# tonyzyl/ladcast

Measured on AMD Instinct MI355X. Metric: ensemble-member-steps/sec, higher is better.
Workload: dtype f32

## Files before the change

### ladcast_amd/csrc/gemm_bf16x3_v3.hip

```cpp
#include <math.h>
#include <stdio.h>
#include <stdlib.h>

#include "common.h"

namespace {

#include "gemm_v3_common.inc"
#include "gemm_v3_kstep_f32.inc"

struct SKArgs {
  DevProblem pr[MAXP];
  int np;
  int G;
  long long U;
  long long tiles;
  float* ws;
  unsigned* counters;
  unsigned upg, urem;
};

__device__ __forceinline__ long long range_start(long long g, const SKArgs& a) {
  const unsigned gu = static_cast<unsigned>(g);
  return static_cast<long long>(gu * a.upg + (gu < a.urem ? gu : a.urem));
}

__device__ __forceinline__ int find_problem_by_unit(const SKArgs& a, long long u) {
  int pi = 0;
#pragma unroll
  for (int k = 1; k < MAXP; ++k)
    if (k < a.np && u >= a.pr[k].unit0) pi = k;
  return pi;
}

#ifdef LDC_GEMM_STAMPS
#define LDC_STAMP(i)                                                                                        \
  if (threadIdx.x == 0)                                                                                     \
    reinterpret_cast<unsigned long long*>(a.counters)[65536 + blockIdx.x * 16 + (i)] = __builtin_amdgcn_s_memrealtime();
#define LDC_STAMP_CLK(i)                                                                                    \
  if (threadIdx.x == 0)                                                                                     \
    reinterpret_cast<unsigned long long*>(a.counters)[65536 + blockIdx.x * 16 + (i)] = __builtin_amdgcn_s_memtime();
#else
#define LDC_STAMP(i)
#define LDC_STAMP_CLK(i)
#endif

template <int BM, int TERMS, bool CONV = false>
__global__ __launch_bounds__(512) void gemm_bf16x3_v3_kernel(SKArgs a) {
  constexpr int CPK = TERMS == 1 ? 2 * BK : BK;
  constexpr int RT = BM / 128;
  constexpr int NACC = RT * 8;
  constexpr int STAGE_B = (BM + BN) * ROW_B;
  constexpr int SLOT_FLOATS = BM * BN;
  constexpr int NAI = BM / 64;
  constexpr int ND = NAI + 2;
  constexpr int NDH = ND / 2;
  extern __shared__ __attribute__((aligned(16))) unsigned char smem[];
  const int wave = __builtin_amdgcn_readfirstlane(static_cast<int>(threadIdx.x) >> 6);
  LDC_STAMP(0)
  int seg_ = 0;
  (void)seg_;
  int g;
  {
    const int bid = blockIdx.x, G = a.G;
    const int q = G >> 3, r = G & 7, xcd = bid & 7;
    g = (xcd < r ? xcd * (q + 1) : r * (q + 1) + (xcd - r) * q) + (bid >> 3);
  }
  auto uniform64 = [](long long v) {
    const unsigned lo = __builtin_amdgcn_readfirstlane(static_cast<unsigned>(v));
    const unsigned hi = __builtin_amdgcn_readfirstlane(static_cast<unsigned>(static_cast<unsigned long long>(v) >> 32));
    return static_cast<long long>((static_cast<unsigned long long>(hi) << 32) | lo);
  };
  const long long u_begin = uniform64(range_start(g, a));
  const long long u_end = uniform64(range_start(g + 1, a));
  const unsigned smem_lds = lds_addr(smem);

  struct Seg {
    int pi, tile, k0, k1, b, bm, bn;
  };
  auto decode = [&](long long u_) {
    Seg sg;
    sg.pi = find_problem_by_unit(a, u_);
    const DevProblem& Q = a.pr[sg.pi];
    const unsigned local = static_cast<unsigned>(u_ - Q.unit0), kt_u = static_cast<unsigned>(Q.kt);
    sg.tile = __builtin_amdgcn_readfirstlane(static_cast<int>(local / kt_u));
    sg.k0 = static_cast<int>(local - static_cast<unsigned>(sg.tile) * kt_u);
    const long long left = u_end - u_;
    sg.k1 = (Q.kt - sg.k0 <= left) ? Q.kt : sg.k0 + static_cast<int>(left);
    const unsigned per_b = static_cast<unsigned>(Q.tm * Q.tn), tile_u = static_cast<unsigned>(sg.tile);
    const unsigned b_ = tile_u / per_b;
    const unsigned t_in = tile_u - b_ * per_b;
    const unsigned strip = static_cast<unsigned>(Q.rm * Q.tn);
    const unsigned sr = t_in / strip;
    const unsigned r_in = t_in - sr * strip;
    const int rest = Q.tm - static_cast<int>(sr) * Q.rm;
    const unsigned h_sr = static_cast<unsigned>(rest < Q.rm ? rest : Q.rm);
    const unsigned bn_ = r_in / h_sr;
    sg.b = __builtin_amdgcn_readfirstlane(static_cast<int>(b_));
    sg.bn = __builtin_amdgcn_readfirstlane(static_cast<int>(bn_));
    sg.bm = __builtin_amdgcn_readfirstlane(static_cast<int>(sr) * Q.rm + static_cast<int>(r_in - bn_ * h_sr));
    return sg;
  };
  auto prefetch_next = [&](const Seg& sg) __attribute__((always_inline)) {
    const DevProblem& Q = a.pr[sg.pi];
    const int ln = fresh_lane();
    const int lr_ = ln >> 3, lp_ = ln & 7;
    const float* __restrict__ An = Q.A + static_cast<long long>(sg.b) * Q.d.a_bs;
    const long long wrb = static_cast<long long>(Q.d.K) * (TERMS == 1 ? 2 : 4);
    unsigned char* dump = smem + NSTAGE * STAGE_B + wave * 1024;
#pragma unroll
    for (int j = 0; j < 2; ++j) {
      const bool live = sg.k0 + j < sg.k1;
      const long long koff = static_cast<long long>(live ? sg.k0 + j : sg.k1 - 1) * (BK * 4);
      unsigned char* sA = smem + j * STAGE_B;
      unsigned char* sW = sA + BM * ROW_B;
#pragma unroll
      for (int i = 0; i < NAI; ++i) {
        const int r = 8 * (wave + 8 * i) + lr_;
        int gm = sg.bm * BM + r;
        gm = gm < Q.d.M ? gm : Q.d.M - 1;
        dma16(reinterpret_cast<const unsigned char*>(An + static_cast<long long>(gm) * Q.d.lda) + ((lp_ ^ swz(r)) << 4) + koff,
              live ? sA + (wave + 8 * i) * 1024 : dump);
      }
#pragma unroll
      for (int i = 0; i < 2; ++i) {
        const int r = 8 * (wave + 8 * i) + lr_;
        int gn = sg.bn * BN + r;
        gn = gn < Q.d.N ? gn : Q.d.N - 1;
        dma16(Q.W + static_cast<long long>(gn) * wrb + ((lp_ ^ swz(r)) << 4) + koff, live ? sW + (wave + 8 * (i)) * 1024 : dump);
      }
    }
  };
  long long u = u_begin;
  Seg cur{};
  if (u < u_end) cur = decode(u);
  bool prefetched = false;
  while (u < u_end) {
    const int pi = cur.pi;
    const DevProblem& P = a.pr[pi];
    const int tile = cur.tile, k0 = cur.k0, k1 = cur.k1, b = cur.b, bm = cur.bm, bn = cur.bn;
    const int lane = fresh_lane();
    const int fr = lane & 15;
    const int kg = lane >> 4;
    const int lr = lane >> 3, lp = lane & 7;
    const unsigned f_r = swz(fr);
    const unsigned off_hi = fr * ROW_B + (((2 * kg) ^ f_r) << 4);
    const unsigned off_lo = fr * ROW_B + (((2 * kg + 1) ^ f_r) << 4);
    const unsigned a_hi = smem_lds + (16 * RT * wave) * ROW_B + off_hi;
    const unsigned a_lo = smem_lds + (16 * RT * wave) * ROW_B + off_lo;
    const unsigned w_hi = smem_lds + BM * ROW_B + off_hi;
    const unsigned w_lo = smem_lds + BM * ROW_B + off_lo;
    const int M = P.d.M, N = P.d.N, K = P.d.K;
    const bool wave_rows = bm * BM + 16 * RT * wave < M;
    const float* __restrict__ A = P.A + static_cast<long long>(b) * P.d.a_bs;
    const int lda = P.d.lda;
    const long long w_row_bytes = static_cast<long long>(K) * (TERMS == 1 ? 2 : 4);

#ifdef LDC_GEMM_STAMPS_PROLOGUE
    if (seg_ == 0) { LDC_STAMP(9) }
#endif
    const unsigned char* a_src[NAI];
    const unsigned char* w_src[2];
    int pix_b[NAI], pix_hw[NAI];
    const int cslot = lp ^ swz(8 * (wave & 1) + lr);
    auto conv_tap_base = [&](int i, int tap) {
      const int ky = tap / P.ks, kx = tap - ky * P.ks;
      const int src = pix_b[i] + ldc_sphere_src_pixel(pix_hw[i] >> 16, pix_hw[i] & 0xffff, ky, kx, P.cH, P.cW, P.ks);
      return reinterpret_cast<const unsigned char*>(A + static_cast<long long>(src) * lda) + (cslot << 4);
    };
#pragma unroll
    for (int i = 0; i < NAI; ++i) {
      const int r = 8 * (wave + 8 * i) + lr;
      int gm = bm * BM + r;
      gm = gm < M ? gm : M - 1;
      if constexpr (CONV) {
        const int hw = P.cH * P.cW;
        const int bimg = gm / hw;
        const int rem = gm - bimg * hw;
        const int h = rem / P.cW;
        pix_b[i] = bimg * hw;
        pix_hw[i] = (h << 16) | (rem - h * P.cW);
        a_src[i] = conv_tap_base(i, k0 >> P.kshift);
      } else {
        a_src[i] = reinterpret_cast<const unsigned char*>(A + static_cast<long long>(gm) * lda) + ((lp ^ swz(r)) << 4);
      }
    }
#pragma unroll
    for (int i = 0; i < 2; ++i) {
      const int r = 8 * (wave + 8 * i) + lr;
      int gn = bn * BN + r;
      gn = gn < N ? gn : N - 1;
      w_src[i] = P.W + static_cast<long long>(gn) * w_row_bytes + ((lp ^ swz(r)) << 4);
    }
    auto issue_one = [&](int kt_, int stage, int i) {
      const bool live = kt_ < k1;
      unsigned char* sA = smem + stage * STAGE_B;
      unsigned char* sW = sA + BM * ROW_B;
      unsigned char* dump = smem + NSTAGE * STAGE_B + wave * 1024;
      const int kt = live ? kt_ : k1 - 1;
      const long long koff = static_cast<long long>(kt) * (BK * 4);
#ifdef LDC_GEMM_DIAG_NODMA
      if (kt >= 0) return;
#endif
      if (i < NAI) {
        if constexpr (CONV) {
          const int chunk = kt & ((1 << P.kshift) - 1);
          if (chunk == 0) a_src[i] = conv_tap_base(i, kt >> P.kshift);
          const unsigned char* src = a_src[i] + chunk * (BK * 4);
          if (chunk * CPK + CPK > P.cin) {
            if (chunk * CPK + (TERMS == 0 ? 4 * cslot : 8 * (TERMS == 3 ? (cslot >> 1) : cslot)) >= P.cin) src = P.zero16;
          }
          dma16(src, live ? sA + (wave + 8 * i) * 1024 : dump);
        } else {
          dma16(a_src[i] + koff, live ? sA + (wave + 8 * i) * 1024 : dump);
        }
      } else {
        dma16(w_src[i - NAI] + koff, live ? sW + (wave + 8 * (i - NAI)) * 1024 : dump);
      }
    };

// ... 77 lines not shown
    const unsigned sb1 = st1 * STAGE_B;                                                                      \
    const unsigned wch = w_hi + sb, wcl = w_lo + sb, wnh = w_hi + sb1, wnl = w_lo + sb1;                     \
    const unsigned anh = a_hi + sb1, anl = a_lo + sb1;                                                       \
    constexpr bool dma2 = true;              \
    constexpr bool dma3 = true;  \
        \
    if constexpr (RT == 2) {                                                                                 \
      asm volatile("s_waitcnt lgkmcnt(6)" : "+v"(AH[0]), "+v"(AL[0]), "+v"(AH[1]), "+v"(AL[1]), "+v"(wh0), "+v"(wl0)); \
    } else {                                                                                                 \
      asm volatile("s_waitcnt lgkmcnt(6)" : "+v"(AH[0]), "+v"(AL[0]), "+v"(wh0), "+v"(wl0));                 \
    }                                                                                                        \
    LDC_SB;                                                                                                  \
    LDC_CT(0, wh0, wl0, AH, AL)                                                                              \
    LDC_RD_W(wh0, wl0, wch, wcl, 4)                                                                                \
    if (dma2) issue_one(kt + 2, st2, NDH + 0);                                                               \
    LDC_WAIT(6, wh1, wl1)                                                                                    \
    LDC_CT(1, wh1, wl1, AH, AL)                                                                              \
    LDC_RD_W(wh1, wl1, wch, wcl, 5)                                                                                \
    if (dma2) issue_one(kt + 2, st2, NDH + 1);                                                               \
    LDC_WAIT(6, wh2, wl2)                                                                                    \
    LDC_CT(2, wh2, wl2, AH, AL)                                                                              \
    LDC_RD_W(wh2, wl2, wch, wcl, 6)                                                                                \
    if constexpr (NDH == 3) {                                                                                \
      if (dma2) issue_one(kt + 2, st2, NDH + 2);                                                             \
    }                                                                                                        \
    LDC_WAIT(6, wh3, wl3)                                                                                    \
    LDC_CT(3, wh3, wl3, AH, AL)                                                                              \
    LDC_RD_W(wh3, wl3, wch, wcl, 7)                                                                          \
    LDC_WAIT(6, wh0, wl0)                                                                                    \
    LDC_CT(4, wh0, wl0, AH, AL)                                                                              \
                                                                         \
    asm volatile("s_waitcnt lgkmcnt(0)" : "+v"(wh1), "+v"(wl1), "+v"(wh2), "+v"(wl2), "+v"(wh3), "+v"(wl3)); \
    if constexpr (ND == 6) {                                                                                 \
      asm volatile("s_waitcnt vmcnt(6)" ::: "memory");                                                       \
    } else {                                                                                                 \
      asm volatile("s_waitcnt vmcnt(4)" ::: "memory");                                                       \
    }                                                                                                        \
    LDC_KSTEP_BARRIER                                                                                        \
    LDC_SB;                                                                                                  \
                          \
    LDC_RD_A(AHN, ALN, anh, anl)                                                                             \
    LDC_RD_W(wh0, wl0, wnh, wnl, 0)                                                                          \
    if (dma3) issue_one(kt + 3, st, 0);                                                                      \
    LDC_SB;                                                                                                  \
    LDC_CT(5, wh1, wl1, AH, AL)                                                                              \
    LDC_RD_W(wh1, wl1, wnh, wnl, 1)                                                                               \
    if (dma3) issue_one(kt + 3, st, 1);                                                                      \
    LDC_SB;                                                                                                  \
    LDC_CT(6, wh2, wl2, AH, AL)                                                                              \
    LDC_RD_W(wh2, wl2, wnh, wnl, 2)                                                                               \
    if constexpr (NDH == 3) {                                                                                \
      if (dma3) issue_one(kt + 3, st, 2);                                                                    \
    }                                                                                                        \
    LDC_SB;                                                                                                  \
    LDC_CT(7, wh3, wl3, AH, AL)                                                                              \
    LDC_RD_W(wh3, wl3, wnh, wnl, 3)                                                                               \
    LDC_SB;                                                                                                  \
    st = st1;                                                                                                \
    sb = sb1;                                                                                                \
  }

#define LDC_MM_ON(ACC, WF, AF, J) LDC_MMF(ACC, WF, AF, J)
#define LDC_MM_OFF(ACC, WF, AF, J)
#if defined(LDC_AB_BUILD) && defined(LDC_GEMM_F32_NO_PAIRS)
  constexpr bool PAIRED = false;
#else
  constexpr bool PAIRED = TERMS == 0 && RT == 1;
#endif

#ifdef LDC_GEMM_STAMPS_PROLOGUE
    if (seg_ == 0) { LDC_STAMP(10) }
#endif
    if (!prefetched) {
#pragma unroll
      for (int i = 0; i < ND; ++i) issue_one(k0, 0, i);
#pragma unroll
      for (int i = 0; i < ND; ++i) issue_one(k0 + 1, 1, i);
    }
#ifdef LDC_GEMM_STAMPS_PROLOGUE
    if (seg_ == 0) { LDC_STAMP(11) }
#endif
    const long long u_next = u + (k1 - k0);
    Seg nxt = cur;
    if (u_next < u_end) nxt = decode(u_next);
    if constexpr (ND == 6) {
      asm volatile("s_waitcnt vmcnt(6)" ::: "memory");
    } else {
      asm volatile("s_waitcnt vmcnt(4)" ::: "memory");
    }
    __builtin_amdgcn_s_barrier();
    LDC_STAMP(1 + 4 * seg_)
    if (seg_ == 0) { LDC_STAMP_CLK(13) }
    if constexpr (PAIRED) {
      LDC_KSTEP_Q_PROLOGUE(ah0, al0)
    } else {
      LDC_RD_A(ah0, al0, a_hi, a_lo)
      LDC_RD_W(wh0, wl0, w_hi, w_lo, 0)
      LDC_RD_W(wh1, wl1, w_hi, w_lo, 1)
      LDC_RD_W(wh2, wl2, w_hi, w_lo, 2)
      LDC_RD_W(wh3, wl3, w_hi, w_lo, 3)
    }
#pragma unroll
    for (int i = 0; i < NDH; ++i) issue_one(k0 + 2, 2, i);
    LDC_SB;

    unsigned sb = 0;
    int st = 0;
    if constexpr (PAIRED) {
      static_assert(!PAIRED || ND == 4, "the interleaved k-step is written for the 128-row tile's 4 DMA pieces");
      if (wave_rows) {
        for (int kt = k0; kt < k1; ++kt) {
          LDC_KSTEP_Q(ah0, al0, ah1, al1, LDC_MM_ON)
          ++kt;
          if (kt >= k1) break;
          LDC_KSTEP_Q(ah1, al1, ah0, al0, LDC_MM_ON)
        }
      } else {
        for (int kt = k0; kt < k1; ++kt) {
          LDC_KSTEP_Q(ah0, al0, ah1, al1, LDC_MM_OFF)
          ++kt;
          if (kt >= k1) break;
          LDC_KSTEP_Q(ah1, al1, ah0, al0, LDC_MM_OFF)
        }
      }
    } else {
      for (int kt = k0; kt < k1; ++kt) {
        LDC_KSTEP(ah0, al0, ah1, al1)
        ++kt;
        if (kt >= k1) break;
        LDC_KSTEP(ah1, al1, ah0, al0)
      }
    }
    asm volatile("s_waitcnt lgkmcnt(0)" : "+v"(wh0), "+v"(wl0), "+v"(wh1), "+v"(wl1), "+v"(wh2), "+v"(wl2), "+v"(wh3), "+v"(wl3));
#pragma unroll
    for (int rt = 0; rt < RT; ++rt) asm volatile("" : "+v"(ah0[rt]), "+v"(al0[rt]), "+v"(ah1[rt]), "+v"(al1[rt]));
#undef LDC_KSTEP
#undef LDC_MM_ON
#undef LDC_MM_OFF
#undef LDC_WAIT
#undef LDC_CT
#undef LDC_MMF
#undef LDC_MM
#undef LDC_RD_A
#undef LDC_RD_W
#undef LDC_SB
    __builtin_amdgcn_s_barrier();
    prefetched = false;
    if constexpr (!CONV && TERMS == 0) {
#if !defined(LDC_GEMM_DIAG_NODMA) && !defined(LDC_GEMM_NO_PREFETCH)
      if (u_next < u_end) {
        prefetch_next(nxt);
        prefetched = true;
      }
#endif
    }
    if (seg_ == 0) { LDC_STAMP_CLK(14) }
    LDC_STAMP(2 + 4 * seg_)

    if (k0 == 0 && k1 == P.kt) {
      tile_epilogue<BM, !CONV, LinearRows<BM>, true, TERMS == 0>(P, b, bm, bn, acc, wave, lane);
    } else {
      const int lane_h = fresh_lane();
      float* slot = a.ws + (static_cast<long long>(2 * g) + (k0 > 0 ? 0 : 1)) * SLOT_FLOATS + lane_h;
#pragma unroll
      for (int i = 0; i < NACC; ++i)
#pragma unroll
        for (int r = 0; r < 4; ++r)
          __hip_atomic_store(slot + ((wave * NACC + i) * 4 + r) * 64, acc[i][r], __ATOMIC_RELAXED, __HIP_MEMORY_SCOPE_AGENT);
      asm volatile("s_waitcnt vmcnt(0)" ::: "memory");
      __builtin_amdgcn_s_barrier();
      const long long f = P.unit0 + static_cast<long long>(tile) * P.kt;
      const long long l = f + P.kt;
      long long g_first = g;
      while (g_first > 0 && range_start(g_first, a) > f) --g_first;
      long long g_last = g;
      while (g_last + 1 < a.G && range_start(g_last + 1, a) < l) ++g_last;
      const unsigned pieces = static_cast<unsigned>(g_last - g_first + 1);
      unsigned* cnt = a.counters + (P.tile0 + tile);
      unsigned* flag = reinterpret_cast<unsigned*>(smem + NSTAGE * STAGE_B);
      if (wave == 0 && lane_h == 0) {
        const unsigned ticket = __hip_atomic_fetch_add(cnt, 1u, __ATOMIC_RELAXED, __HIP_MEMORY_SCOPE_AGENT);
        const unsigned last = (ticket == pieces - 1) ? 1u : 0u;
        if (last) {
          __builtin_amdgcn_fence(__ATOMIC_ACQUIRE, "agent");
          asm volatile("s_waitcnt vmcnt(0)" ::: "memory");
          __hip_atomic_store(cnt, 0u, __ATOMIC_RELAXED, __HIP_MEMORY_SCOPE_AGENT);
        }
        *flag = last;
      }
      __syncthreads();
      LDC_STAMP(3 + 4 * seg_)
      const unsigned is_last = *flag;
      __syncthreads();
      if (is_last) {
#pragma unroll
        for (int i = 0; i < NACC; ++i) acc[i] = f32x4{0.f, 0.f, 0.f, 0.f};
        for (long long gp = g_first; gp <= g_last; ++gp) {
          const long long s = range_start(gp, a);
          const float* sl = a.ws + (2 * gp + (s > f ? 0 : 1)) * SLOT_FLOATS;
#pragma unroll
          for (int i = 0; i < NACC; ++i) {
#pragma unroll
            for (int r = 0; r < 4; ++r) acc[i][r] += sl[((wave * NACC + i) * 4 + r) * 64 + lane_h];
          }
        }
        tile_epilogue<BM, !CONV, LinearRows<BM>, true, TERMS == 0>(P, b, bm, bn, acc, wave, lane);
      }
    }
    u = u_next;
    cur = nxt;
    LDC_STAMP(4 + 4 * seg_)
#ifdef LDC_GEMM_STAMPS
    if (seg_ < 2) ++seg_;
#endif
  }
  LDC_STAMP(15)
}

struct ConvParams {
  int H, W, cin, ks, kshift;
};

constexpr int LDC_SPLIT_GROUP = -100;

template <int BM, int TERMS, bool CONV = false>
int launch_v3(const ldc_gemm_problem* problems, const ldc_qkv_epilogue* epi, int n, void* workspace, long long workspace_bytes,
              void* stream, const ConvParams* cp = nullptr, bool may_split_group = false) {
  constexpr int SLOT_FLOATS = BM * BN;
  constexpr int STAGE_B = (BM + BN) * ROW_B;
  constexpr int CUS = 256;
  SKArgs a{};
  a.np = n;
  long long U = 0, tiles = 0;
  for (int i = 0; i < n; ++i) {
    const ldc_gemm_problem& q = problems[i];
    LDC_CHECK_PTR(q.A);
    LDC_CHECK_PTR(q.W);
    LDC_CHECK_PTR(q.C);
    const ldc_gemm_desc& d = q.d;
    if (d.M <= 0 || d.N <= 0 || d.K <= 0 || d.batch <= 0) return LDC_ERR_ARG;
    if (d.K % (TERMS == 1 ? 2 * BK : BK)) return LDC_ERR_UNSUPPORTED;
    if constexpr (TERMS == 0) {
      if (d.flags != 0 || d.ldw != d.K) return LDC_ERR_UNSUPPORTED;
    } else {
      if (!(d.flags & LDC_GEMM_A_SPLIT)) return LDC_ERR_UNSUPPORTED;
    }
    LDC_CHECK_ALIGN16(q.A);
    LDC_CHECK_ALIGN16(q.W);
    if constexpr (TERMS == 0) {
      if ((d.lda & 3) || (d.a_bs & 3)) return LDC_ERR_UNSUPPORTED;
    } else {
      if ((d.lda & 7) || (d.a_bs & 7) || (reinterpret_cast<unsigned long long>(q.A) & 31ull)) return LDC_ERR_ALIGN;
    }
    if (d.act < LDC_ACT_NONE || d.act > LDC_ACT_RELU) return LDC_ERR_UNSUPPORTED;
    DevProblem& P = a.pr[i];
    P.A = q.A;
    P.W = reinterpret_cast<const unsigned char*>(q.W);
    P.bias = q.bias;
    P.gate = q.gate;
    P.R = q.R;
    P.C = q.C;
    P.d = d;
    {
      auto al16 = [](const void* q_) { return (reinterpret_cast<unsigned long long>(q_) & 15ull) == 0; };
      bool v4 = (d.N % 4 == 0) && (d.ldc % 4 == 0) && (d.c_bs % 4 == 0) && al16(q.C);
      if (q.bias) v4 = v4 && al16(q.bias);
      if (q.gate) v4 = v4 && al16(q.gate) && (d.gate_bs % 4 == 0);
      if (q.R) v4 = v4 && al16(q.R) && (d.ldr % 4 == 0) && (d.r_bs % 4 == 0);
      P.vec4 = v4 ? 1 : 0;
      P.c_split = (TERMS != 0 && (d.flags & LDC_GEMM_C_SPLIT)) ? (TERMS == 3 ? LDC_FMT_SPLIT : LDC_FMT_BF16) : 0;
      if (P.c_split && !(v4 && d.ldc % 8 == 0 && d.ldc >= ((d.N + 7) & ~7) &&
                         d.c_bs % 8 == 0 && (reinterpret_cast<unsigned long long>(q.C) & 31ull) == 0))
        return LDC_ERR_ALIGN;
    }
    if (epi != nullptr && epi[i].heads > 0) {
      const ldc_qkv_epilogue& e = epi[i];
      auto al16 = [](const void* q_) { return (reinterpret_cast<unsigned long long>(q_) & 15ull) == 0; };
      if (d.N != 3 * e.heads * BN || d.act != LDC_ACT_NONE || q.gate != nullptr || q.R != nullptr) return LDC_ERR_ARG;
      if ((e.wq == nullptr) != (e.wk == nullptr) || e.reserved != nullptr || e.rope_row0 < 0) return LDC_ERR_ARG;
      if constexpr (TERMS == 0) {
        if ((d.ldc & 3) || (d.c_bs & 3) || !al16(q.C)) return LDC_ERR_ALIGN;
      } else {
        if ((d.ldc & 7) || (d.c_bs & 7) || (reinterpret_cast<unsigned long long>(q.C) & 31ull)) return LDC_ERR_ALIGN;
      }
      if (!al16(e.wq) || !al16(e.wk) || !al16(e.rope) || (q.bias && !al16(q.bias))) return LDC_ERR_ALIGN;
      P.qkv_heads = e.heads;
      P.rope_row0 = e.rope_row0;
      P.qk_w[0] = e.wq;
      P.qk_w[1] = e.wk;
      P.rope_cs = e.rope;
      P.eps = e.eps;
      P.qscale = e.qscale != 0.f ? e.qscale : 0.08838834764831845f * 1.4426950408889634f;
    }
    if constexpr (CONV) {
      P.cH = cp->H; P.cW = cp->W; P.cin = cp->cin; P.ks = cp->ks; P.kshift = cp->kshift;
      P.zero16 = static_cast<const unsigned char*>(workspace) + LDC_GEMM_COUNTER_BYTES - 64;
    }
    P.tm = ldc_cdiv(d.M, BM);
    P.tn = ldc_cdiv(d.N, BN);
    P.kt = d.K / (TERMS == 1 ? 2 * BK : BK);
// ... 12 lines not shown
      }
      if (const char* e = LDC_AB_GETENV("LDC_BF16X3_RM")) {
        const int f = atoi(e);
        if (f >= 0) P.rm = (f == 0 || f > P.tm) ? P.tm : f;
      }
    }
    const long long t = static_cast<long long>(d.batch) * P.tm * P.tn;
    tiles += t;
    U += t * P.kt;
  }
  if (tiles > LDC_GEMM_COUNTER_BYTES / 4 - 16) return LDC_ERR_UNSUPPORTED;
  const long long slot_bytes = SLOT_FLOATS * static_cast<long long>(sizeof(float));
  long long G = CUS;
  {
    bool same_kt = true;
    for (int i = 1; i < n; ++i) same_kt = same_kt && (a.pr[i].kt == a.pr[0].kt);
    long long best = 0;
    if (same_kt) {
      const int kt = a.pr[0].kt;
      double best_score = 0.0;
      for (int sfac = 1; sfac <= 8; ++sfac) {
        if (kt % sfac || (sfac > 1 && kt / sfac < 8)) continue;
        const long long items = tiles * sfac;
        long long gd = items < CUS ? items : CUS;
        while (gd > 1 && items % gd) --gd;
        const double score = static_cast<double>(gd) * (1.0 - 0.02 * (sfac - 1));
        if (score > best_score) {
          best_score = score;
          best = gd;
        }
      }
    }
    long long few = 0;
    if (same_kt && best < 160) {
      const int kt = a.pr[0].kt;
      for (int sfac = 8; sfac >= 2; --sfac)
        if (kt % sfac == 0 && kt / sfac >= 8 && tiles * sfac <= CUS) {
          few = tiles * sfac;
          break;
        }
    }
    if (may_split_group && TERMS != 0 && n > 1 && best < 160 && few == 0) return LDC_SPLIT_GROUP;
    if (best >= 160) {
      G = best;
    } else if (few > 0) {
      G = few;
    } else {
      const double kt_avg = static_cast<double>(U) / static_cast<double>(tiles);
      long long umin = static_cast<long long>(sqrt(kt_avg * 8.0) + 0.5);
      if (umin < 1) umin = 1;
      const long long gmax = U / umin > 0 ? U / umin : 1;
      if (gmax < G) G = gmax;
    }
  }
  if constexpr (TERMS == 0) {
    if (U >= 4 * CUS) G = CUS;
  }
  static const char* const force_g = LDC_AB_GETENV("LDC_BF16X3_G");
  if (force_g) {
    const long long g_ = atoll(force_g);
    if (g_ > 0 && g_ <= CUS) G = g_;
  }
  if (U < G) G = U;
  if (workspace == nullptr) return LDC_ERR_ARG;
  if (workspace_bytes < LDC_GEMM_COUNTER_BYTES + 2 * slot_bytes) return LDC_ERR_ARG;
  {
    const long long fit = (workspace_bytes - LDC_GEMM_COUNTER_BYTES) / (2 * slot_bytes);
    if (fit < G) G = fit;
  }
  LDC_CHECK_ALIGN16(workspace);
  if (U >= (1LL << 31)) return LDC_ERR_UNSUPPORTED;
#ifdef LDC_AB_BUILD
  {
    static const bool dbg = getenv("LDC_GEMM_DEBUG_G") != nullptr;
    if (dbg)
      fprintf(stderr, "ldc_gemm cut: terms %d conv %d n %d tiles %lld kt0 %d BM %d G %lld U %lld %s\n", TERMS, int(CONV), n, tiles, a.pr[0].kt, BM, G, U,
              (U % G == 0 && (U / G) % a.pr[0].kt == 0) ? "whole tiles" : (U % G == 0 ? "equal ranges" : "UNALIGNED"));
  }
#endif
  a.G = static_cast<int>(G);
  a.U = U;
  a.upg = static_cast<unsigned>(U / G);
  a.urem = static_cast<unsigned>(U % G);
  a.tiles = tiles;
  a.ws = reinterpret_cast<float*>(static_cast<unsigned char*>(workspace) + LDC_GEMM_COUNTER_BYTES);
  a.counters = static_cast<unsigned*>(workspace);
  const size_t lds = NSTAGE * STAGE_B + 8 * 1024;
  static const bool attr_set = [&] {
    (void)hipFuncSetAttribute(reinterpret_cast<const void*>(gemm_bf16x3_v3_kernel<BM, TERMS, CONV>),
                              hipFuncAttributeMaxDynamicSharedMemorySize, static_cast<int>(lds));
    return true;
  }();
  (void)attr_set;
  hipLaunchKernelGGL((gemm_bf16x3_v3_kernel<BM, TERMS, CONV>), dim3(a.G), dim3(512), lds, static_cast<hipStream_t>(stream), a);
  return ldc_launch_status();
}

}

static int gemm_v3_dispatch(const ldc_gemm_problem* problems, const ldc_qkv_epilogue* epi, int n, void* workspace,
                            long long workspace_bytes, void* stream) {
  LDC_CHECK_PTR(problems);
  if (n <= 0 || n > MAXP) return LDC_ERR_ARG;
  long long tiles256 = 0;
  for (int i = 0; i < n; ++i) {
    const ldc_gemm_desc& d = problems[i].d;
    if (d.M <= 0 || d.N <= 0 || d.batch <= 0) return LDC_ERR_ARG;
    if (!(d.flags & LDC_GEMM_A_SPLIT)) return LDC_ERR_UNSUPPORTED;
    if (((d.flags ^ problems[0].d.flags) & LDC_GEMM_BF16_1TERM) != 0) return LDC_ERR_ARG;
    tiles256 += static_cast<long long>(d.batch) * ldc_cdiv(d.M, 256) * ldc_cdiv(d.N, BN);
  }
  static const char* const force_thr = LDC_AB_GETENV("LDC_BF16X3_SMALL_TILES");
  bool small = tiles256 < (force_thr ? atoll(force_thr) : 400);
  static const char* const force_bm = LDC_AB_GETENV("LDC_BF16X3_BM");
  if (force_bm) small = (atoi(force_bm) == 128);
  const bool one = (problems[0].d.flags & LDC_GEMM_BF16_1TERM) != 0;
  auto launch = [&](const ldc_gemm_problem* pr, const ldc_qkv_epilogue* ep, int cnt, bool sm, bool may_split) {
    if (one)
      return sm ? launch_v3<128, 1>(pr, ep, cnt, workspace, workspace_bytes, stream, nullptr, may_split)
                : launch_v3<256, 1>(pr, ep, cnt, workspace, workspace_bytes, stream, nullptr, may_split);
    return sm ? launch_v3<128, 3>(pr, ep, cnt, workspace, workspace_bytes, stream, nullptr, may_split)
              : launch_v3<256, 3>(pr, ep, cnt, workspace, workspace_bytes, stream, nullptr, may_split);
  };
  const int st = launch(problems, epi, n, small, true);
  if (st != LDC_SPLIT_GROUP) return st;
  for (int i = 0; i < n; ++i) {
    const ldc_gemm_desc& d = problems[i].d;
    bool sm = static_cast<long long>(d.batch) * ldc_cdiv(d.M, 256) * ldc_cdiv(d.N, BN) < (force_thr ? atoll(force_thr) : 400);
    if (force_bm) sm = (atoi(force_bm) == 128);
    const int sti = launch(problems + i, epi ? epi + i : nullptr, 1, sm, false);
    if (sti != LDC_OK) return sti;
  }
  return LDC_OK;
}

static int gemm_f32_ring(const ldc_gemm_problem* problems, const ldc_qkv_epilogue* epi, int n, void* workspace, long long workspace_bytes,
                         void* stream) {
  LDC_CHECK_PTR(problems);
  if (n <= 0 || n > MAXP) return LDC_ERR_ARG;
  for (int i = 0; i < n; ++i)
    if (problems[i].d.flags & LDC_GEMM_F32_REGSTAGE) return LDC_ERR_UNSUPPORTED;
  auto al16 = [](const void* q_) { return q_ != nullptr && (reinterpret_cast<unsigned long long>(q_) & 15ull) == 0; };
  if (!al16(workspace) || workspace_bytes < LDC_GEMM_COUNTER_BYTES + 2ll * 256 * BN * static_cast<long long>(sizeof(float)))
    return LDC_ERR_UNSUPPORTED;
  for (int i = 0; i < n; ++i) {
    const ldc_gemm_desc& d = problems[i].d;
    if (d.M <= 0 || d.N <= 0 || d.K <= 0 || d.batch <= 0) return LDC_ERR_ARG;
    if (!al16(problems[i].A) || !al16(problems[i].W)) return LDC_ERR_UNSUPPORTED;
  }
#ifdef LDC_AB_BUILD
  static const char* const force_bm = getenv("LDC_F32_RING_BM");
  if (force_bm && atoi(force_bm) == 256) return launch_v3<256, 0>(problems, epi, n, workspace, workspace_bytes, stream);
#endif
  return launch_v3<128, 0>(problems, epi, n, workspace, workspace_bytes, stream);
}

int ldc_gemm_grouped_f32_ring(const ldc_gemm_problem* problems, int n, void* workspace, long long workspace_bytes, void* stream) {
  return gemm_f32_ring(problems, nullptr, n, workspace, workspace_bytes, stream);
}

extern "C" int ldc_gemm_grouped_qkv_f32(const ldc_gemm_problem* problems, const ldc_qkv_epilogue* epi, int n, void* workspace,
                                        long long workspace_bytes, void* stream) {
  LDC_CHECK_PTR(epi);
  return gemm_f32_ring(problems, epi, n, workspace, workspace_bytes, stream);
}

int ldc_gemm_grouped_bf16x3_v3(const ldc_gemm_problem* problems, int n, void* workspace, long long workspace_bytes,
                               void* stream) {
  return gemm_v3_dispatch(problems, nullptr, n, workspace, workspace_bytes, stream);
}
// ... 69 lines not shown
```

### ladcast_amd/csrc/gemm_streamk.hip

```cpp
#include <math.h>
#include <stdlib.h>
#include <string.h>

#include "common.h"

namespace {

constexpr int BM = 128, BN = 128, BK = 32;
constexpr int LDP = 36;
constexpr int STAGE_FLOATS = (BM + BN) * LDP;
constexpr int SLOT_FLOATS = BM * BN;
constexpr int MAXP = LDC_GEMM_MAX_PROBLEMS;

struct DevProblem {
  const float* A;
  const float* W;
  const float* bias;
  const float* gate;
  const float* R;
  float* C;
  ldc_gemm_desc d;
  int tm, tn, kt;
  long long unit0;
  long long tile0;
// ... 314 lines not shown
      unsigned char* As = smem_b + stage * STAGE_BYTES_B;
      unsigned char* Bs = As + BM * PITCH_B;
      uint4 h, l;
      split8(ra00, ra01, h, l);
      *reinterpret_cast<uint4*>(As + srow0 * PITCH_B + skc * 16) = h;
      *reinterpret_cast<uint4*>(As + srow0 * PITCH_B + 64 + skc * 16) = l;
      split8(ra10, ra11, h, l);
      *reinterpret_cast<uint4*>(As + srow1 * PITCH_B + skc * 16) = h;
      *reinterpret_cast<uint4*>(As + srow1 * PITCH_B + 64 + skc * 16) = l;
      *reinterpret_cast<uint4*>(Bs + srow0 * PITCH_B + skc * 16) = rw00;
      *reinterpret_cast<uint4*>(Bs + srow0 * PITCH_B + 64 + skc * 16) = rw01;
      *reinterpret_cast<uint4*>(Bs + srow1 * PITCH_B + skc * 16) = rw10;
      *reinterpret_cast<uint4*>(Bs + srow1 * PITCH_B + 64 + skc * 16) = rw11;
    };

    f32x16 acc[2][2];
#pragma unroll
    for (int i = 0; i < 2; ++i)
#pragma unroll
      for (int j = 0; j < 2; ++j)
#pragma unroll
        for (int r = 0; r < 16; ++r) acc[i][j][r] = 0.f;

    gload(k0);
    sstore(0);
    __syncthreads();
    for (int kt = k0; kt < k1; ++kt) {
      const int st = (kt - k0) & 1;
      if (kt + 1 < k1) gload(kt + 1);
      const unsigned char* As = smem_b + st * STAGE_BYTES_B;
      const unsigned char* Bs = As + BM * PITCH_B;
      const unsigned char* a_base = As + (wm * 64 + frag_row) * PITCH_B + frag_h * 16;
      const unsigned char* b_base = Bs + (wn * 64 + frag_row) * PITCH_B + frag_h * 16;
#pragma unroll
      for (int s2 = 0; s2 < 2; ++s2) {
        const bf16x8 ah0 = *reinterpret_cast<const bf16x8*>(a_base + s2 * 32);
        const bf16x8 al0 = *reinterpret_cast<const bf16x8*>(a_base + 64 + s2 * 32);
        const bf16x8 ah1 = *reinterpret_cast<const bf16x8*>(a_base + 32 * PITCH_B + s2 * 32);
        const bf16x8 al1 = *reinterpret_cast<const bf16x8*>(a_base + 32 * PITCH_B + 64 + s2 * 32);
        const bf16x8 wh0 = *reinterpret_cast<const bf16x8*>(b_base + s2 * 32);
        const bf16x8 wl0 = *reinterpret_cast<const bf16x8*>(b_base + 64 + s2 * 32);
        const bf16x8 wh1 = *reinterpret_cast<const bf16x8*>(b_base + 32 * PITCH_B + s2 * 32);
        const bf16x8 wl1 = *reinterpret_cast<const bf16x8*>(b_base + 32 * PITCH_B + 64 + s2 * 32);
#define LDC_MFMA3(ACC, AH, AL, WH, WL)                                        \
  ACC = __builtin_amdgcn_mfma_f32_32x32x16_bf16(AL, WH, ACC, 0, 0, 0);        \
  ACC = __builtin_amdgcn_mfma_f32_32x32x16_bf16(AH, WL, ACC, 0, 0, 0);        \
  ACC = __builtin_amdgcn_mfma_f32_32x32x16_bf16(AH, WH, ACC, 0, 0, 0);
        LDC_MFMA3(acc[0][0], ah0, al0, wh0, wl0)
        LDC_MFMA3(acc[0][1], ah0, al0, wh1, wl1)
        LDC_MFMA3(acc[1][0], ah1, al1, wh0, wl0)
        LDC_MFMA3(acc[1][1], ah1, al1, wh1, wl1)
      }
      if (kt + 1 < k1) sstore(st ^ 1);
      __syncthreads();
    }

    if (k0 == 0 && k1 == P.kt) {
      tile_epilogue(P, b, bm, bn, acc, wm, wn, lane);
    } else {
      publish_or_reduce(a, P, g, tile, k0, b, bm, bn, acc, wave, wm, wn, lane, reinterpret_cast<unsigned*>(smem_b));
    }
    u += k1 - k0;
  }
}

__global__ __launch_bounds__(256) void pack_weight_bf16x2_kernel(const float* __restrict__ W, uint4* __restrict__ out,
                                                                 int N, int K, int ldw) {
  const long long idx = static_cast<long long>(blockIdx.x) * 256 + threadIdx.x;
  const int kchunks = K >> 3;
  if (idx >= static_cast<long long>(N) * kchunks) return;
  const int n = static_cast<int>(idx / kchunks), kc = static_cast<int>(idx - static_cast<long long>(n) * kchunks);
  const float4* src = reinterpret_cast<const float4*>(W + static_cast<long long>(n) * ldw + kc * 8);
  uint4 h, l;
  split8(src[0], src[1], h, l);
  out[idx * 2] = h;
  out[idx * 2 + 1] = l;
}

}

extern "C" int ldc_sizeof_gemm_problem(void) { return static_cast<int>(sizeof(ldc_gemm_problem)); }

extern "C" long long ldc_gemm_grouped_workspace_bytes(void) {
  return LDC_GEMM_COUNTER_BYTES + 2LL * 512 * SLOT_FLOATS * static_cast<long long>(sizeof(float));
}

extern "C" int ldc_gemm_grouped_workspace_init(void* workspace, long long workspace_bytes, void* stream) {
  LDC_CHECK_PTR(workspace);
  if (workspace_bytes < LDC_GEMM_COUNTER_BYTES) return LDC_ERR_ARG;
  hipError_t e = hipMemsetAsync(workspace, 0, LDC_GEMM_COUNTER_BYTES, static_cast<hipStream_t>(stream));
  return e == hipSuccess ? LDC_OK : -(1000 + static_cast<int>(e));
}

static int gemm_grouped_impl(const ldc_gemm_problem* problems, int n, void* workspace, long long workspace_bytes,
                             void* stream, bool split_bf16) {
  LDC_CHECK_PTR(problems);
  if (n <= 0 || n > MAXP) return LDC_ERR_ARG;
  SKArgs a{};
  a.np = n;
  long long U = 0, tiles = 0;
  for (int i = 0; i < n; ++i) {
    const ldc_gemm_problem& q = problems[i];
    LDC_CHECK_PTR(q.A);
    LDC_CHECK_PTR(q.W);
    LDC_CHECK_PTR(q.C);
    const ldc_gemm_desc& d = q.d;
    if (d.M <= 0 || d.N <= 0 || d.K <= 0 || d.batch <= 0) return LDC_ERR_ARG;
    LDC_CHECK_ALIGN16(q.A);
    LDC_CHECK_ALIGN16(q.W);
    if ((d.K & 3) || (d.lda & 3) || (d.a_bs & 3)) return LDC_ERR_ALIGN;
    if (split_bf16 ? (d.K & 7) != 0 : (d.ldw & 3) != 0) return LDC_ERR_ALIGN;
    if (d.act < LDC_ACT_NONE || d.act > LDC_ACT_RELU) return LDC_ERR_UNSUPPORTED;
    if ((d.flags & ~LDC_GEMM_F32_REGSTAGE) != 0) return LDC_ERR_UNSUPPORTED;
    DevProblem& P = a.pr[i];
    P.A = q.A;
    P.W = q.W;
    P.bias = q.bias;
    P.gate = q.gate;
    P.R = q.R;
    P.C = q.C;
    P.d = d;
    P.tm = ldc_cdiv(d.M, BM);
    P.tn = ldc_cdiv(d.N, BN);
    P.kt = ldc_cdiv(d.K, BK);
    P.unit0 = U;
    P.tile0 = tiles;
    const long long t = static_cast<long long>(d.batch) * P.tm * P.tn;
    tiles += t;
    U += t * P.kt;
  }
  if (tiles > LDC_GEMM_COUNTER_BYTES / 4 - 16) return LDC_ERR_UNSUPPORTED;
  const long long slot_bytes = SLOT_FLOATS * static_cast<long long>(sizeof(float));
  long long G = 512;
  {
    const double kt_avg = static_cast<double>(U) / static_cast<double>(tiles);
    long long umin = static_cast<long long>(sqrt(kt_avg * (split_bf16 ? 7.0 : 2.0)) + 0.5);
    if (umin < 1) umin = 1;
    const long long gmax = U / umin > 0 ? U / umin : 1;
    if (gmax < G) G = gmax;
  }
  if (U < G) G = U;
  if (workspace == nullptr || workspace_bytes < LDC_GEMM_COUNTER_BYTES + 2 * slot_bytes) return LDC_ERR_ARG;
  {
    const long long fit = (workspace_bytes - LDC_GEMM_COUNTER_BYTES) / (2 * slot_bytes);
    if (fit < G) G = fit;
  }
  LDC_CHECK_ALIGN16(workspace);
  a.G = static_cast<int>(G);
  a.U = U;
  a.tiles = tiles;
  a.ws = reinterpret_cast<float*>(static_cast<unsigned char*>(workspace) + LDC_GEMM_COUNTER_BYTES);
  a.counters = static_cast<unsigned*>(workspace);
  const size_t lds = split_bf16 ? 2 * STAGE_BYTES_B : 2 * STAGE_FLOATS * sizeof(float);
  static const bool attr_set = [&] {
    (void)hipFuncSetAttribute(reinterpret_cast<const void*>(gemm_streamk_kernel),
                              hipFuncAttributeMaxDynamicSharedMemorySize, static_cast<int>(2 * STAGE_FLOATS * sizeof(float)));
    (void)hipFuncSetAttribute(reinterpret_cast<const void*>(gemm_streamk_bf16x3_kernel),
                              hipFuncAttributeMaxDynamicSharedMemorySize, 2 * STAGE_BYTES_B);
    return true;
  }();
  (void)attr_set;
  hipStream_t s = static_cast<hipStream_t>(stream);
  if (split_bf16) hipLaunchKernelGGL(gemm_streamk_bf16x3_kernel, dim3(a.G), dim3(256), lds, s, a);
  else hipLaunchKernelGGL(gemm_streamk_kernel, dim3(a.G), dim3(256), lds, s, a);
  return ldc_launch_status();
}

// ... 67 lines not shown
```

Measured before the change: 3.178.

## Add dynamic work-stealing tail chunks to stream-K bf16x3 GEMM

Reserves the last portion of each workgroup's stream-K unit range as small fixed-size chunks. Workgroups that finish early claim these through per-XCD atomic cursors, hopping across XCDs when their local pool is empty. The goal is to cut load imbalance at the end of the persistent GEMM. In exchange it adds atomics, extra partial-sum slots, and a larger workspace, and the fixup now scans every chunk to count pieces and reduce them. Cursor reset depends on the last workgroup finishing.

Measured after the change: 2.966. 0.933x the previous value.

```diff
diff --git a/ladcast_amd/csrc/gemm_bf16x3_v3.hip b/ladcast_amd/csrc/gemm_bf16x3_v3.hip
--- a/ladcast_amd/csrc/gemm_bf16x3_v3.hip
+++ b/ladcast_amd/csrc/gemm_bf16x3_v3.hip
@@ -18,11 +18,25 @@
   float* ws;
   unsigned* counters;
   unsigned upg, urem;
+  unsigned tn, ps, npc;
+  int fixed;
+  unsigned* cursors;
 };
 
 __device__ __forceinline__ long long range_start(long long g, const SKArgs& a) {
   const unsigned gu = static_cast<unsigned>(g);
   return static_cast<long long>(gu * a.upg + (gu < a.urem ? gu : a.urem));
+}
+
+__device__ __forceinline__ void chunk_bounds(const SKArgs& a, int gp, int j, long long& b, long long& e) {
+  const long long re = range_start(gp + 1, a);
+  if (j < 0) {
+    b = range_start(gp, a);
+    e = re - a.tn;
+  } else {
+    b = re - a.tn + static_cast<long long>(static_cast<unsigned>(j) * a.ps);
+    e = b + a.ps;
+  }
 }
 
 __device__ __forceinline__ int find_problem_by_unit(const SKArgs& a, long long u) {
@@ -55,6 +69,7 @@
   constexpr int NAI = BM / 64;
   constexpr int ND = NAI + 2;
   constexpr int NDH = ND / 2;
+  constexpr bool TAIL = TERMS == 0 && !CONV && BM == 128;
   extern __shared__ __attribute__((aligned(16))) unsigned char smem[];
   const int wave = __builtin_amdgcn_readfirstlane(static_cast<int>(threadIdx.x) >> 6);
   LDC_STAMP(0)
@@ -78,7 +93,7 @@
   struct Seg {
     int pi, tile, k0, k1, b, bm, bn;
   };
-  auto decode = [&](long long u_) {
+  auto decode = [&](long long u_, long long u_end) {
     Seg sg;
     sg.pi = find_problem_by_unit(a, u_);
     const DevProblem& Q = a.pr[sg.pi];
@@ -132,10 +147,52 @@
     }
   };
   long long u = u_begin;
+  long long ue = u_end, cb = u_begin;
+  int cr = g, cj = -1;
+  const bool tail_on = TAIL && a.npc > 0;
+  unsigned claim_v = 0;
+  int cx = blockIdx.x & 7, hops = 0;
+  unsigned fixed_next = 0;
+  unsigned* claim_lds = reinterpret_cast<unsigned*>(smem + NSTAGE * STAGE_B + 8 * 1024);
+  (void)claim_lds; (void)fixed_next; (void)hops; (void)cx; (void)claim_v; (void)cb; (void)cj;
+  auto issue_claim = [&]() {
+    if (a.fixed) claim_v = fixed_next++;
+    else if (threadIdx.x == 0) claim_v = __hip_atomic_fetch_add(a.cursors + cx, 1u, __ATOMIC_RELAXED, __HIP_MEMORY_SCOPE_AGENT);
+  };
+  auto resolve_claim = [&](int& pr_, int& pj_) -> bool {
+    unsigned ci = __builtin_amdgcn_readfirstlane(*reinterpret_cast<volatile unsigned*>(claim_lds));
+    if (a.fixed) {
+      pr_ = g;
+      pj_ = static_cast<int>(ci);
+      return ci < a.npc;
+    }
+    const unsigned nr = static_cast<unsigned>(a.G) >> 3, cnt = nr * a.npc;
+    while (ci >= cnt) {
+      if (++hops == 8) return false;
+      cx = (cx + 1) & 7;
+      __syncthreads();
+      if (threadIdx.x == 0) *claim_lds = __hip_atomic_fetch_add(a.cursors + cx, 1u, __ATOMIC_RELAXED, __HIP_MEMORY_SCOPE_AGENT);
+      __syncthreads();
+      ci = __builtin_amdgcn_readfirstlane(*reinterpret_cast<volatile unsigned*>(claim_lds));
+    }
+    const unsigned j = ci / nr;
+    pr_ = static_cast<int>(static_cast<unsigned>(cx) * nr + (ci - j * nr));
+    pj_ = static_cast<int>(j);
+    return true;
+  };
+#ifdef LDC_GEMM_STAMPS
+  unsigned long long taken_ = 0;
+#endif
+  if constexpr (TAIL) {
+    if (tail_on) {
+      ue = u_end - a.tn;
+      issue_claim();
+    }
+  }
   Seg cur{};
-  if (u < u_end) cur = decode(u);
+  if (u < ue) cur = decode(u, ue);
   bool prefetched = false;
-  while (u < u_end) {
+  for (bool have = u < ue; have;) {
     const int pi = cur.pi;
     const DevProblem& P = a.pr[pi];
     const int tile = cur.tile, k0 = cur.k0, k1 = cur.k1, b = cur.b, bm = cur.bm, bn = cur.bn;
@@ -379,7 +436,8 @@
 #endif
     const long long u_next = u + (k1 - k0);
     Seg nxt = cur;
-    if (u_next < u_end) nxt = decode(u_next);
+    bool more = u_next < ue;
+    if (more) nxt = decode(u_next, ue);
     if constexpr (ND == 6) {
       asm volatile("s_waitcnt vmcnt(6)" ::: "memory");
     } else {
@@ -441,11 +499,38 @@
 #undef LDC_RD_A
 #undef LDC_RD_W
 #undef LDC_SB
+    if constexpr (TAIL) {
+      if (tail_on && !more) {
+        if (threadIdx.x == 0) *claim_lds = claim_v;
+        asm volatile("s_waitcnt lgkmcnt(0)" ::: "memory");
+      }
+    }
     __builtin_amdgcn_s_barrier();
     prefetched = false;
+    long long nu = u_next, nue = ue, ncb = cb;
+    int ncr = cr, ncj = cj;
+    if constexpr (TAIL) {
+      if (tail_on && !more) {
+        int pr_, pj_;
+        if (resolve_claim(pr_, pj_)) {
+          chunk_bounds(a, pr_, pj_, ncb, nue);
+          ncb = uniform64(ncb);
+          nue = uniform64(nue);
+          nu = ncb;
+          ncr = pr_;
+          ncj = pj_;
+          nxt = decode(nu, nue);
+          more = true;
+          issue_claim();
+#ifdef LDC_GEMM_STAMPS
+          taken_ += 1ull + ((static_cast<unsigned>(pr_) / (static_cast<unsigned>(a.G) >> 3) != (blockIdx.x & 7u)) ? (1ull << 32) : 0ull);
+#endif
+        }
+      }
+    }
     if constexpr (!CONV && TERMS == 0) {
 #if !defined(LDC_GEMM_DIAG_NODMA) && !defined(LDC_GEMM_NO_PREFETCH)
-      if (u_next < u_end) {
+      if (more) {
         prefetch_next(nxt);
         prefetched = true;
       }
@@ -458,7 +543,11 @@
       tile_epilogue<BM, !CONV, LinearRows<BM>, true, TERMS == 0>(P, b, bm, bn, acc, wave, lane);
     } else {
       const int lane_h = fresh_lane();
-      float* slot = a.ws + (static_cast<long long>(2 * g) + (k0 > 0 ? 0 : 1)) * SLOT_FLOATS + lane_h;
+      long long sidx = static_cast<long long>(2 * cr) + (k0 > 0 ? 0 : 1);
+      if constexpr (TAIL) {
+        if (cj >= 0) sidx = u == cb ? static_cast<long long>(2 * a.G) + static_cast<long long>(cr) * a.npc + cj : static_cast<long long>(2 * a.G) + static_cast<long long>(a.G) * a.npc + cr;
+      }
+      float* slot = a.ws + sidx * SLOT_FLOATS + lane_h;
 #pragma unroll
       for (int i = 0; i < NACC; ++i)
 #pragma unroll
@@ -468,11 +557,20 @@
       __builtin_amdgcn_s_barrier();
       const long long f = P.unit0 + static_cast<long long>(tile) * P.kt;
       const long long l = f + P.kt;
-      long long g_first = g;
+      long long g_first = cr;
       while (g_first > 0 && range_start(g_first, a) > f) --g_first;
-      long long g_last = g;
+      long long g_last = cr;
       while (g_last + 1 < a.G && range_start(g_last + 1, a) < l) ++g_last;
-      const unsigned pieces = static_cast<unsigned>(g_last - g_first + 1);
+      unsigned pieces = static_cast<unsigned>(g_last - g_first + 1);
+      if constexpr (TAIL) {
+        pieces = 0;
+        for (long long gp = g_first; gp <= g_last; ++gp)
+          for (int j = -1; j < static_cast<int>(a.npc); ++j) {
+            long long b_, e_;
+            chunk_bounds(a, static_cast<int>(gp), j, b_, e_);
+            if ((b_ > f ? b_ : f) < (e_ < l ? e_ : l)) ++pieces;
+          }
+      }
       unsigned* cnt = a.counters + (P.tile0 + tile);
       unsigned* flag = reinterpret_cast<unsigned*>(smem + NSTAGE * STAGE_B);
       if (wave == 0 && lane_h == 0) {
@@ -492,6 +590,22 @@
       if (is_last) {
 #pragma unroll
         for (int i = 0; i < NACC; ++i) acc[i] = f32x4{0.f, 0.f, 0.f, 0.f};
+        if constexpr (TAIL) {
+          for (long long gp = g_first; gp <= g_last; ++gp)
+            for (int j = -1; j < static_cast<int>(a.npc); ++j) {
+              long long b_, e_;
+              chunk_bounds(a, static_cast<int>(gp), j, b_, e_);
+              if ((b_ > f ? b_ : f) >= (e_ < l ? e_ : l)) continue;
+              const long long si = j < 0 ? 2 * gp + (b_ > f ? 0 : 1)
+                                         : (b_ >= f ? 2LL * a.G + gp * a.npc + j : 2LL * a.G + static_cast<long long>(a.G) * a.npc + gp);
+              const float* sl = a.ws + si * SLOT_FLOATS;
+#pragma unroll
+              for (int i = 0; i < NACC; ++i) {
+#pragma unroll
+                for (int r = 0; r < 4; ++r) acc[i][r] += sl[((wave * NACC + i) * 4 + r) * 64 + lane_h];
+              }
+            }
+        } else {
         for (long long gp = g_first; gp <= g_last; ++gp) {
           const long long s = range_start(gp, a);
           const float* sl = a.ws + (2 * gp + (s > f ? 0 : 1)) * SLOT_FLOATS;
@@ -501,18 +615,43 @@
             for (int r = 0; r < 4; ++r) acc[i][r] += sl[((wave * NACC + i) * 4 + r) * 64 + lane_h];
           }
         }
+        }
         tile_epilogue<BM, !CONV, LinearRows<BM>, true, TERMS == 0>(P, b, bm, bn, acc, wave, lane);
       }
     }
-    u = u_next;
+    u = nu;
+    ue = nue;
+    cb = ncb;
+    cr = ncr;
+    cj = ncj;
     cur = nxt;
+    have = more;
     LDC_STAMP(4 + 4 * seg_)
 #ifdef LDC_GEMM_STAMPS
     if (seg_ < 2) ++seg_;
 #endif
   }
+  if constexpr (TAIL) {
+    if (tail_on && !a.fixed && threadIdx.x == 0) {
+      const unsigned t = __hip_atomic_fetch_add(a.cursors + 8, 1u, __ATOMIC_RELAXED, __HIP_MEMORY_SCOPE_AGENT);
+      if (t == static_cast<unsigned>(a.G) - 1u) {
+#pragma unroll
+        for (int i = 0; i < 9; ++i) __hip_atomic_store(a.cursors + i, 0u, __ATOMIC_RELAXED, __HIP_MEMORY_SCOPE_AGENT);
+      }
+    }
+#ifdef LDC_GEMM_STAMPS
+    if (threadIdx.x == 0) reinterpret_cast<unsigned long long*>(a.counters)[65536 + 256 * 16 + blockIdx.x] = taken_;
+#endif
+  }
   LDC_STAMP(15)
 }
+
+#ifndef LDC_TAIL_PCT
+#define LDC_TAIL_PCT 12.0
+#endif
+#ifndef LDC_TAIL_PS
+#define LDC_TAIL_PS 8
+#endif
 
 struct ConvParams {
   int H, W, cin, ks, kshift;
@@ -691,10 +830,33 @@
   a.U = U;
   a.upg = static_cast<unsigned>(U / G);
   a.urem = static_cast<unsigned>(U % G);
+  a.cursors = static_cast<unsigned*>(workspace) + (LDC_GEMM_COUNTER_BYTES / 4 - 32);
+  if constexpr (TERMS == 0 && !CONV && BM == 128) {
+    static const char* const e_pct = LDC_AB_GETENV("LDC_GEMM_TAIL_PCT");
+    static const char* const e_ps = LDC_AB_GETENV("LDC_GEMM_TAIL_PS");
+    static const char* const e_fixed = LDC_AB_GETENV("LDC_GEMM_TAIL_FIXED");
+    const double pct = e_pct ? atof(e_pct) : LDC_TAIL_PCT;
+    const long long ps = e_ps && atoll(e_ps) > 0 ? atoll(e_ps) : LDC_TAIL_PS;
+    if (U >= 4 * CUS && G == CUS && pct > 0.0 && tiles <= LDC_GEMM_COUNTER_BYTES / 4 - 32) {
+      long long kt_min = a.pr[0].kt;
+      for (int i = 1; i < n; ++i) kt_min = a.pr[i].kt < kt_min ? a.pr[i].kt : kt_min;
+      const long long upg = U / G;
+      long long npc = static_cast<long long>(static_cast<double>(upg) * pct / 100.0 / static_cast<double>(ps) + 0.5);
+      const long long slots = (workspace_bytes - LDC_GEMM_COUNTER_BYTES) / slot_bytes;
+      if (npc > slots / G - 3) npc = slots / G - 3;
+      while (npc > 0 && (npc * ps > kt_min || 2 * npc * ps > upg)) --npc;
+      if (npc >= 2) {
+        a.npc = static_cast<unsigned>(npc);
+        a.ps = static_cast<unsigned>(ps);
+        a.tn = a.npc * a.ps;
+        a.fixed = (e_fixed && atoi(e_fixed) != 0) ? 1 : 0;
+      }
+    }
+  }
   a.tiles = tiles;
   a.ws = reinterpret_cast<float*>(static_cast<unsigned char*>(workspace) + LDC_GEMM_COUNTER_BYTES);
   a.counters = static_cast<unsigned*>(workspace);
-  const size_t lds = NSTAGE * STAGE_B + 8 * 1024;
+  const size_t lds = NSTAGE * STAGE_B + 8 * 1024 + ((TERMS == 0 && !CONV && BM == 128) ? 64 : 0);
   static const bool attr_set = [&] {
     (void)hipFuncSetAttribute(reinterpret_cast<const void*>(gemm_bf16x3_v3_kernel<BM, TERMS, CONV>),
                               hipFuncAttributeMaxDynamicSharedMemorySize, static_cast<int>(lds));
diff --git a/ladcast_amd/csrc/gemm_streamk.hip b/ladcast_amd/csrc/gemm_streamk.hip
--- a/ladcast_amd/csrc/gemm_streamk.hip
+++ b/ladcast_amd/csrc/gemm_streamk.hip
@@ -420,7 +420,7 @@
 extern "C" int ldc_sizeof_gemm_problem(void) { return static_cast<int>(sizeof(ldc_gemm_problem)); }
 
 extern "C" long long ldc_gemm_grouped_workspace_bytes(void) {
-  return LDC_GEMM_COUNTER_BYTES + 2LL * 512 * SLOT_FLOATS * static_cast<long long>(sizeof(float));
+  return LDC_GEMM_COUNTER_BYTES + 2LL * 1024 * SLOT_FLOATS * static_cast<long long>(sizeof(float));
 }
 
 extern "C" int ldc_gemm_grouped_workspace_init(void* workspace, long long workspace_bytes, void* stream) {
```
